# nexus-xyz/nexus-zkvm

Hardware: NVIDIA B200
Metric: RISC-V cycles proved/sec @ 2^20 rows (higher is better)
Workload: dtype u32 (M31)

## Files before the change

### nexus_zkvm_b200/csrc/jit.cu

```cuda
#include "pcs.h"
#include "jit.h"
#include <dlfcn.h>
#include <unistd.h>
#include <cstring>
#include <cstdio>
#include <nvrtc.h>
#include <sstream>
#include <cstdlib>

namespace nb {

static u32 jit_bound() {
  static u32 v = 0;
  if (!v) { v = JIT_BLOCK; if (const char* e = getenv("NB200_JIT_BOUND")) { int x = atoi(e); if (x == 256 || x == 512 || x == 1024) v = (u32)x; } }
  return v;
}


namespace {
struct Nvrtc {
  void* h = nullptr;
  nvrtcResult (*CreateProgram)(nvrtcProgram*, const char*, const char*, int, const char* const*, const char* const*) = nullptr;
  nvrtcResult (*CompileProgram)(nvrtcProgram, int, const char* const*) = nullptr;
  nvrtcResult (*GetCUBINSize)(nvrtcProgram, size_t*) = nullptr;
  nvrtcResult (*GetCUBIN)(nvrtcProgram, char*) = nullptr;
  nvrtcResult (*GetProgramLogSize)(nvrtcProgram, size_t*) = nullptr;
  nvrtcResult (*GetProgramLog)(nvrtcProgram, char*) = nullptr;
  nvrtcResult (*DestroyProgram)(nvrtcProgram*) = nullptr;
  bool ok = false;
};
Nvrtc& nvrtc() {
  static Nvrtc n;
  static bool tried = false;
  if (tried) return n;
  tried = true;
  const char* names[] = {"libnvrtc.so.12", "libnvrtc.so", "/usr/local/cuda/lib64/libnvrtc.so.12"};
  for (const char* nm : names) { n.h = dlopen(nm, RTLD_NOW | RTLD_LOCAL); if (n.h) break; }
  if (!n.h) return n;
#define NB_SYM(f) n.f = (decltype(n.f))dlsym(n.h, "nvrtc" #f); if (!n.f) return n;
  NB_SYM(CreateProgram) NB_SYM(CompileProgram) NB_SYM(GetCUBINSize) NB_SYM(GetCUBIN) NB_SYM(GetProgramLogSize) NB_SYM(GetProgramLog) NB_SYM(DestroyProgram)
#undef NB_SYM
  n.ok = true;
  return n;
}

const char* kPrelude = R"SRC(
typedef unsigned int u32; typedef unsigned long long u64;
#define P31 0x7fffffffu
struct Q { u32 c0, c1, c2, c3; };
__device__ __forceinline__ u32 mn(u32 a, u32 b) { return a < b ? a : b; }
__device__ __forceinline__ u32 add(u32 a, u32 b) { u32 s = a + b; return mn(s, s - P31); }
__device__ __forceinline__ u32 sub(u32 a, u32 b) { u32 d = a - b; return mn(d, d + P31); }
__device__ __forceinline__ u32 neg(u32 a) { return a ? P31 - a : 0u; }
// one product: a * 2b = hi * 2^32 + lo  =>  a * b = hi * 2^31 + lo / 2 == hi + lo / 2 (mod P), below 2P
__device__ __forceinline__ u32 mul2(u32 a, u32 b2) { u64 p = (u64)a * (u64)b2; u32 s = (u32)(p >> 32) + ((u32)p >> 1); return mn(s, s - P31); }
__device__ __forceinline__ u32 mul(u32 a, u32 b) { return mul2(a, b + b); }
// canonical residue of any 64-bit value: 2^32 == 2 and 2^31 == 1 (mod P)
__device__ __forceinline__ u32 red64(u64 x) {
  u64 y;                                                // y = 2 * hi + lo < 3 * 2^32 (mad.wide keeps NVVM from expanding it into a carry chain)
  asm("mad.wide.u32 %0, %1, 2, %2;" : "=l"(y) : "r"((u32)(x >> 32)), "l"((u64)(u32)x));
  u32 yl = (u32)y, yh = (u32)(y >> 32);
  u32 s = (yl & P31) + __funnelshift_r(yl, yh, 31);     // <= P + 5
  return mn(s, s - P31);
}
__device__ __forceinline__ Q qadd(Q x, Q y) { return Q{add(x.c0, y.c0), add(x.c1, y.c1), add(x.c2, y.c2), add(x.c3, y.c3)}; }
__device__ __forceinline__ Q qsub(Q x, Q y) { return Q{sub(x.c0, y.c0), sub(x.c1, y.c1), sub(x.c2, y.c2), sub(x.c3, y.c3)}; }
__device__ __forceinline__ Q qneg(Q x) { return Q{neg(x.c0), neg(x.c1), neg(x.c2), neg(x.c3)}; }
__device__ __forceinline__ Q qmulb(Q x, u32 b) { u32 b2 = b + b; return Q{mul2(x.c0, b2), mul2(x.c1, b2), mul2(x.c2, b2), mul2(x.c3, b2)}; }
__device__ __forceinline__ Q qaddb(Q x, u32 b) { x.c0 = add(x.c0, b); return x; }
__device__ __forceinline__ Q qsubb(Q x, u32 b) { x.c0 = sub(x.c0, b); return x; }
// acc + x * y in QM31 with every coordinate accumulated in 64 bits and reduced once.  (a + bu)(c + du) = (ac + R bd) + (ad + bc)u,
// R = 2 + i (the formula of m31.cuh qm31_mul), regrouped per coordinate of x so that each output is four products:
//   r0 = x0 y0 - x1 y1 + x2 (2 y2 - y3) - x3 (y2 + 2 y3)      r1 = x0 y1 + x1 y0 + x2 (y2 + 2 y3) + x3 (2 y2 - y3)
//   r2 = x0 y2 - x1 y3 + x2 y0 - x3 y1                        r3 = x0 y3 + x1 y2 + x2 y1 + x3 y0
// ny1 = P - y1, ny3 = P - y3, g = 2 y2 - y3, gp = y2 + 2 y3, h = P - gp: all <= P, so 4 products + acc < 2^64.
__device__ __forceinline__ Q qmac(Q acc, Q x, u32 y0, u32 y1, u32 y2, u32 y3, u32 ny1, u32 ny3, u32 g, u32 gp, u32 h) {
  u64 r0 = (u64)acc.c0 + (u64)x.c0 * y0 + (u64)x.c1 * ny1 + (u64)x.c2 * g + (u64)x.c3 * h;
  u64 r1 = (u64)acc.c1 + (u64)x.c0 * y1 + (u64)x.c1 * y0 + (u64)x.c2 * gp + (u64)x.c3 * g;
  u64 r2 = (u64)acc.c2 + (u64)x.c0 * y2 + (u64)x.c1 * ny3 + (u64)x.c2 * y0 + (u64)x.c3 * ny1;
  u64 r3 = (u64)acc.c3 + (u64)x.c0 * y3 + (u64)x.c1 * y2 + (u64)x.c2 * y1 + (u64)x.c3 * y0;
  return Q{red64(r0), red64(r1), red64(r2), red64(r3)};
}
__device__ __forceinline__ Q qmul(Q x, Q y) {
  u32 gp = add(add(y.c3, y.c3), y.c2), g = sub(add(y.c2, y.c2), y.c3);
  return qmac(Q{0u, 0u, 0u, 0u}, x, y.c0, y.c1, y.c2, y.c3, P31 - y.c1, P31 - y.c3, g, gp, P31 - gp);
}
// x^(P-2): 30 squarings + 8 products
__device__ __forceinline__ u32 sqn(u32 x, int n) { for (int i = 0; i < n; ++i) x = mul(x, x); return x; }
__device__ __forceinline__ u32 minv(u32 x) {
  u32 a2 = mul(sqn(x, 1), x), a4 = mul(sqn(a2, 2), a2), a8 = mul(sqn(a4, 4), a4), a16 = mul(sqn(a8, 8), a8);
  u32 a24 = mul(sqn(a16, 8), a8), a28 = mul(sqn(a24, 4), a4), a29 = mul(sqn(a28, 1), x);
  return mul(sqn(a29, 2), x);
}
// (a + bu)^-1 = (a - bu) / (a^2 - (2 + i) b^2), a, b in CM31 (the formula of m31.cuh qm31_inv); the CM31 inverse is conj / norm
__device__ __noinline__ Q qinv(Q q) {
  u32 b2r = sub(mul(q.c2, q.c2), mul(q.c3, q.c3)), b2i = mul(add(q.c2, q.c2), q.c3);           // b^2
  u32 a2r = sub(mul(q.c0, q.c0), mul(q.c1, q.c1)), a2i = mul(add(q.c0, q.c0), q.c1);           // a^2
  u32 dr = sub(a2r, sub(add(b2r, b2r), b2i)), di = sub(a2i, add(add(b2i, b2i), b2r));          // a^2 - (2 b^2 + i b^2)
  u32 ni = minv(add(mul(dr, dr), mul(di, di)));
  u32 ir = mul(dr, ni), ii = neg(mul(di, ni));                                                 // 1 / denom
  return Q{sub(mul(q.c0, ir), mul(q.c1, ii)), add(mul(q.c0, ii), mul(q.c1, ir)),
           neg(sub(mul(q.c2, ir), mul(q.c3, ii))), neg(add(mul(q.c2, ii), mul(q.c3, ir)))};
}
__device__ __forceinline__ Q ldq(const u32* p) { uint4 v = __ldg(reinterpret_cast<const uint4*>(p)); return Q{v.x, v.y, v.z, v.w}; }
// rr + coeff * x with the coefficient's derived multipliers precomputed by the host (12 words per constraint, see jit_coeff_table)
__device__ __forceinline__ Q qmac_tab(Q acc, Q x, const u32* t) {
  uint4 a = __ldg(reinterpret_cast<const uint4*>(t)), b = __ldg(reinterpret_cast<const uint4*>(t) + 1), c = __ldg(reinterpret_cast<const uint4*>(t) + 2);
  return qmac(acc, x, a.x, a.y, a.z, a.w, b.x, b.y, b.z, b.w, c.x);
}
)SRC";

template <class Ld>
void emit_op(std::ostringstream& o, const AirInstr& in, Ld ld) {
  switch (in.op) {
    case OP_LOADM: o << "b[" << in.dst << "] = " << ld(in.a) << ";"; break;
    case OP_CONSTB: o << "b[" << in.dst << "] = " << in.a << "u;"; break;
    case OP_ADDB: o << "b[" << in.dst << "] = add(b[" << in.a << "], b[" << in.b << "]);"; break;
    case OP_SUBB: o << "b[" << in.dst << "] = sub(b[" << in.a << "], b[" << in.b << "]);"; break;
    case OP_MULB: o << "b[" << in.dst << "] = mul(b[" << in.a << "], b[" << in.b << "]);"; break;
    case OP_NEGB: o << "b[" << in.dst << "] = neg(b[" << in.a << "]);"; break;
    case OP_PARAME: o << "e[" << in.dst << "] = ldq(params + " << 4 * in.a << ");"; break;
    case OP_ADDE: o << "e[" << in.dst << "] = qadd(e[" << in.a << "], e[" << in.b << "]);"; break;
    case OP_SUBE: o << "e[" << in.dst << "] = qsub(e[" << in.a << "], e[" << in.b << "]);"; break;
    case OP_MULE: o << "e[" << in.dst << "] = qmul(e[" << in.a << "], e[" << in.b << "]);"; break;
    case OP_NEGE: o << "e[" << in.dst << "] = qneg(e[" << in.a << "]);"; break;
    case OP_ADDEB: o << "e[" << in.dst << "] = qaddb(e[" << in.a << "], b[" << in.b << "]);"; break;
    case OP_SUBEB: o << "e[" << in.dst << "] = qsubb(e[" << in.a << "], b[" << in.b << "]);"; break;
    case OP_MULEB: o << "e[" << in.dst << "] = qmulb(e[" << in.a << "], b[" << in.b << "]);"; break;
    case OP_BTOE: o << "e[" << in.dst << "] = Q{b[" << in.a << "], 0u, 0u, 0u};"; break;
    case OP_LOADME: o << "e[" << in.dst << "] = Q{" << ld(in.a) << ", " << ld(in.a + 1) << ", " << ld(in.a + 2) << ", " << ld(in.a + 3) << "};"; break;
    default: break;
  }
}

struct ChunkLive { std::vector<std::vector<u32>> in_b, in_e, out_b, out_e; };
static void instr_regs(const AirInstr& in, std::vector<u32>& rb, std::vector<u32>& re, int& wb, int& we) {
  wb = we = -1;
  switch (in.op) {
    case OP_LOADM: case OP_CONSTB: wb = (int)in.dst; break;
    case OP_ADDB: case OP_SUBB: case OP_MULB: rb = {in.a, in.b}; wb = (int)in.dst; break;
    case OP_NEGB: rb = {in.a}; wb = (int)in.dst; break;
    case OP_PARAME: case OP_LOADME: we = (int)in.dst; break;
    case OP_ADDE: case OP_SUBE: case OP_MULE: re = {in.a, in.b}; we = (int)in.dst; break;
    case OP_NEGE: re = {in.a}; we = (int)in.dst; break;
    case OP_ADDEB: case OP_SUBEB: case OP_MULEB: re = {in.a}; rb = {in.b}; we = (int)in.dst; break;
    case OP_BTOE: rb = {in.a}; we = (int)in.dst; break;
    case OP_CONSTRB: rb = {in.a}; break;
    case OP_CONSTRE: re = {in.a}; break;
    case OP_FRAC: re = {in.a, in.b}; break;
    default: break;
  }
}
static ChunkLive chunk_liveness(const std::vector<AirInstr>& prog, size_t CH, u32 nb, u32 ne) {
  const size_t n_chunks = (prog.size() + CH - 1) / CH;
  ChunkLive L; L.in_b.resize(n_chunks); L.in_e.resize(n_chunks); L.out_b.resize(n_chunks); L.out_e.resize(n_chunks);
  std::vector<char> lb(nb + 1, 0), le(ne + 1, 0);
  std::vector<std::vector<char>> after_b(n_chunks), after_e(n_chunks);
  for (size_t ci = n_chunks; ci-- > 0;) {
    after_b[ci] = lb; after_e[ci] = le;
    for (size_t pc = std::min(prog.size(), (ci + 1) * CH); pc-- > ci * CH;) {
      std::vector<u32> rb, re; int wb, we;
      instr_regs(prog[pc], rb, re, wb, we);
      if (wb >= 0) lb[wb] = 0;
      if (we >= 0) le[we] = 0;
      for (u32 r : rb) lb[r] = 1;
      for (u32 r : re) le[r] = 1;
    }
    for (u32 r = 0; r < nb; ++r) if (lb[r]) L.in_b[ci].push_back(r);
    for (u32 r = 0; r < ne; ++r) if (le[r]) L.in_e[ci].push_back(r);
  }
  for (size_t ci = 0; ci < n_chunks; ++ci) {
    std::vector<char> wrb(nb + 1, 0), wre(ne + 1, 0);
    for (size_t pc = ci * CH; pc < std::min(prog.size(), (ci + 1) * CH); ++pc) {
      std::vector<u32> rb, re; int wb, we;
      instr_regs(prog[pc], rb, re, wb, we);
      if (wb >= 0) wrb[wb] = 1;
      if (we >= 0) wre[we] = 1;
    }
    for (u32 r = 0; r < nb; ++r) if (wrb[r] && after_b[ci][r]) L.out_b[ci].push_back(r);
    for (u32 r = 0; r < ne; ++r) if (wre[r] && after_e[ci][r]) L.out_e[ci].push_back(r);
  }
  return L;
}

std::string gen_source(const AirComponent& c) {
  std::ostringstream o;
  o << kPrelude;
  const u32 DL = c.log_size;
  o << "__device__ __forceinline__ u32 offrow(u32 i, int off, u32 EL) { const u32 DL = " << DL << ";\n"
    << "  u32 prev = __brev(i) >> (32 - EL); u32 half = 1u << (EL - 1); long long step = (long long)off * (1ll << (EL - DL - 1)); long long v;\n"
    << "  if (prev < half) { v = ((long long)prev + step) % (long long)half; if (v < 0) v += half; }\n"
    << "  else { v = ((long long)prev - step) % (long long)half; if (v < 0) v += half; v += half; }\n"
    << "  return __brev((u32)v) >> (32 - EL); }\n";
  const u32 nb = c.n_base_regs ? c.n_base_regs : 1, ne = c.n_ext_regs ? c.n_ext_regs : 1;
  o << "struct St { u32 b[" << nb << "]; Q e[" << ne << "]; Q rr; };\n";
  o << "#define NB_NMASKS " << c.masks.size() << "\n__constant__ const u32* ccols[NB_NMASKS > 0 ? NB_NMASKS : 1];\n";
  auto ld = [&](u32 m) {
    std::ostringstream s;
    if (c.masks[m].off == 0) s << "__ldg(ccols[" << m << "] + row)";
    else s << "__ldg(ccols[" << m << "] + offrow(row, " << c.masks[m].off << ", EL))";
    return s.str();
  };
  size_t CH = 250;
  if (const char* e = getenv("NB200_JIT_CHUNK")) { long v = atol(e); if (v >= 16 && v <= 100000) CH = (size_t)v; }
  size_t n_chunks = (c.prog.size() + CH - 1) / CH;
  const ChunkLive live = chunk_liveness(c.prog, CH, nb, ne);
  u32 k = 0;
  for (size_t ci = 0; ci < n_chunks; ++ci) {
    o << "__device__ __noinline__ void chunk" << ci << "(St& s, const u32* const* __restrict__ cols, const u32* __restrict__ params, const u32* __restrict__ coeff, u32 row, u32 EL) {\n";
    o << "  u32 b[" << nb << "]; Q e[" << ne << "]; Q rr = s.rr;\n";
    for (u32 r : live.in_b[ci]) o << "  b[" << r << "] = s.b[" << r << "];";
    for (u32 r : live.in_e[ci]) o << "  e[" << r << "] = s.e[" << r << "];";
    o << "\n";
    for (size_t pc = ci * CH; pc < std::min(c.prog.size(), (ci + 1) * CH); ++pc) {
      const AirInstr& in = c.prog[pc];
      o << "  ";
      switch (in.op) {
        case OP_CONSTRB: o << "rr = qadd(rr, qmulb(ldq(coeff + " << JIT_COEFF_WORDS * k << "), b[" << in.a << "]));"; ++k; break;
        case OP_CONSTRE: o << "rr = qmac_tab(rr, e[" << in.a << "], coeff + " << JIT_COEFF_WORDS * k << ");"; ++k; break;
        default: emit_op(o, in, ld); break;
      }
      o << "\n";
    }
    for (u32 r : live.out_b[ci]) o << "  s.b[" << r << "] = b[" << r << "];";
    for (u32 r : live.out_e[ci]) o << "  s.e[" << r << "] = e[" << r << "];";
    o << "\n  s.rr = rr;\n}\n";
  }
  o << "extern \"C\" __global__ void __launch_bounds__(" << jit_bound() << ", 1) nbjit(const u32* const* __restrict__ cols, const u32* __restrict__ params, const u32* __restrict__ coeff,\n"
    << "    const u32* __restrict__ dinv, u32* __restrict__ a0, u32* __restrict__ a1, u32* __restrict__ a2, u32* __restrict__ a3, u32 EL, u32 row0) {\n"
    << "  const u32 row = row0 + blockIdx.x * blockDim.x + threadIdx.x;   // row0: a rank of a multi-GPU proof evaluates its slice of the domain's rows\n  St s;\n"
    << "  for (int i = 0; i < " << nb << "; ++i) s.b[i] = 0u;\n  for (int i = 0; i < " << ne << "; ++i) s.e[i] = Q{0u, 0u, 0u, 0u};\n  s.rr = Q{0u, 0u, 0u, 0u};\n";
  for (size_t ci = 0; ci < n_chunks; ++ci) o << "  chunk" << ci << "(s, cols, params, coeff, row, EL);\n  __syncthreads();\n";
  o << "  const u32 di = __ldg(dinv + (row >> " << DL << "));\n"
    << "  a0[row] = add(a0[row], mul(s.rr.c0, di)); a1[row] = add(a1[row], mul(s.rr.c1, di));\n"
    << "  a2[row] = add(a2[row], mul(s.rr.c2, di)); a3[row] = add(a3[row], mul(s.rr.c3, di));\n}\n";
  return o.str();
}

std::string gen_logup_source(const AirComponent& c) {
  std::ostringstream o;
  o << kPrelude;
  const u32 nb = c.lg_base_regs ? c.lg_base_regs : 1, ne = c.lg_ext_regs ? c.lg_ext_regs : 1;
  o << "struct St { u32 b[" << nb << "]; Q e[" << ne << "]; Q fn, fd, run; };\n";
  o << "#define NB_NMASKS " << c.masks.size() << "\n__constant__ const u32* ccols[NB_NMASKS > 0 ? NB_NMASKS : 1];\n";
  auto ld = [&](u32 m) {
    std::ostringstream s;
    if (m < c.masks.size() && c.masks[m].off == 0 && c.masks[m].tree != 2) s << "__ldg(ccols[" << m << "] + row)";
    else s << "0u";
    return s.str();
  };
  size_t CH = 150;
  size_t n_chunks = (c.logup_prog.size() + CH - 1) / CH;
  const ChunkLive live = chunk_liveness(c.logup_prog, CH, nb, ne);
  const int G = 4;
  u32 k = 0; bool have = false; u32 cur_batch = 0;
  std::vector<u32> pending;
  auto flush = [&](std::ostringstream& o2) {
    const int n = (int)pending.size();
    if (n == 0) return;
    o2 << "  {\n";
    for (int g = 1; g < n; ++g) o2 << "    Q pp" << g << " = qmul(" << (g == 1 ? std::string("pfd0") : "pp" + std::to_string(g - 1)) << ", pfd" << g << ");\n";
    o2 << "    Q iv = qinv(" << (n == 1 ? std::string("pfd0") : "pp" + std::to_string(n - 1)) << ");\n";
    for (int g = n - 1; g >= 1; --g)
      o2 << "    { Q t = qmul(iv, " << (g == 1 ? std::string("pfd0") : "pp" + std::to_string(g - 1)) << "); iv = qmul(iv, pfd" << g << "); pfd" << g << " = t; }\n";
    o2 << "    pfd0 = iv;\n";
    for (int g = 0; g < n; ++g) {
      o2 << "    run = qadd(run, qmul(pfn" << g << ", pfd" << g << "));\n";
      for (int cc = 0; cc < 4; ++cc) o2 << "    out[(" << (4 * (size_t)pending[g] + cc) << "ull << LS) + row] = run.c" << cc << ";\n";
    }
    o2 << "  }\n";
    pending.clear();
  };
  auto finalize = [&](std::ostringstream& o2) {
    o2 << "  pfn" << pending.size() << " = fn; pfd" << pending.size() << " = fd;\n";
    pending.push_back(cur_batch);
    if ((int)pending.size() == G) flush(o2);
  };
  o << "struct Pend { Q n[" << G << "], d[" << G << "]; };\n";
  for (size_t ci = 0; ci < n_chunks; ++ci) {
    o << "__device__ __noinline__ void chunk" << ci << "(St& s, Pend& pe, const u32* const* __restrict__ cols, const u32* __restrict__ params, u32* __restrict__ out, u32 row, u32 LS) {\n";
    o << "  u32 b[" << nb << "]; Q e[" << ne << "]; Q fn = s.fn, fd = s.fd, run = s.run;\n";
    for (int g = 0; g < G; ++g) o << "  Q pfn" << g << " = pe.n[" << g << "], pfd" << g << " = pe.d[" << g << "];\n";
    for (u32 r : live.in_b[ci]) o << "  b[" << r << "] = s.b[" << r << "];";
    for (u32 r : live.in_e[ci]) o << "  e[" << r << "] = s.e[" << r << "];";
    o << "\n";
    for (size_t pc = ci * CH; pc < std::min(c.logup_prog.size(), (ci + 1) * CH); ++pc) {
      const AirInstr& in = c.logup_prog[pc];
      if (in.op == OP_FRAC) {
        u32 bt = c.batching[k];
        if (have && bt != cur_batch) { finalize(o); have = false; }
        if (!have) o << "  fn = e[" << in.a << "]; fd = e[" << in.b << "];\n";
        else o << "  fn = qadd(qmul(fn, e[" << in.b << "]), qmul(e[" << in.a << "], fd)); fd = qmul(fd, e[" << in.b << "]);\n";
        cur_batch = bt; have = true; ++k;
      } else {
        o << "  "; emit_op(o, in, ld); o << "\n";
      }
    }
    if (ci + 1 == n_chunks) { if (have) finalize(o); flush(o); }
    for (u32 r : live.out_b[ci]) o << "  s.b[" << r << "] = b[" << r << "];";
    for (u32 r : live.out_e[ci]) o << "  s.e[" << r << "] = e[" << r << "];";
    o << "\n  s.fn = fn; s.fd = fd; s.run = run;\n";
    for (int g = 0; g < G; ++g) o << "  pe.n[" << g << "] = pfn" << g << "; pe.d[" << g << "] = pfd" << g << ";\n";
    o << "}\n";
  }
  o << "extern \"C\" __global__ void __launch_bounds__(" << JIT_BLOCK << ", 1) nbjit(const u32* const* __restrict__ cols, const u32* __restrict__ params, u32* __restrict__ out, u32 LS) {\n"
    << "  const u32 row = blockIdx.x * blockDim.x + threadIdx.x;\n  St s;\n"
    << "  for (int i = 0; i < " << nb << "; ++i) s.b[i] = 0u;\n  for (int i = 0; i < " << ne << "; ++i) s.e[i] = Q{0u, 0u, 0u, 0u};\n"
    << "  s.fn = Q{0u, 0u, 0u, 0u}; s.fd = Q{1u, 0u, 0u, 0u}; s.run = Q{0u, 0u, 0u, 0u};\n"
    << "  Pend pe; for (int i = 0; i < " << 4 << "; ++i) { pe.n[i] = Q{0u, 0u, 0u, 0u}; pe.d[i] = Q{1u, 0u, 0u, 0u}; }\n";
  for (size_t ci = 0; ci < n_chunks; ++ci) o << "  chunk" << ci << "(s, pe, cols, params, out, row, LS);\n  __syncthreads();\n";
  o << "}\n";
  return o.str();
}
}

std::string jit_source(const AirComponent& c) { return gen_source(c); }
std::string jit_logup_source(const AirComponent& c) { return gen_logup_source(c); }

static u32 jit_block() {
  static u32 b = 0;
  if (!b) { b = 512; if (const char* e = getenv("NB200_JIT_BLOCK")) { int v = atoi(e); if (v == 256 || v == 512 || v == 1024) b = (u32)v; } }
  return b < jit_bound() ? b : jit_bound();
}

bool jit_enabled() {
  const char* e = getenv("NB200_JIT");
  return !(e && e[0] == '0');
}

void jit_release(JitKernel& jk) {
  if (jk.lib) cudaLibraryUnload((cudaLibrary_t)jk.lib);
  jk = JitKernel();
}

static nb200_status jit_compile_source(nb200_ctx* ctx, const AirComponent& c, const std::string& src, JitKernel* out);
nb200_status jit_compile_constraints(nb200_ctx* ctx, const AirComponent& c, JitKernel* out) { return jit_compile_source(ctx, c, gen_source(c), out); }
nb200_status jit_compile_logup(nb200_ctx* ctx, const AirComponent& c, JitKernel* out) { return jit_compile_source(ctx, c, gen_logup_source(c), out); }
uint64_t jit_source_key(const std::string& src) {
  uint64_t h = 1469598103934665603ull;
  auto mix = [&](const char* p, size_t n) { for (size_t i = 0; i < n; ++i) { h ^= (unsigned char)p[i]; h *= 1099511628211ull; } };
  mix(src.data(), src.size());
  const char* tgt = "|sm_100a|nb200-jit-4";
  mix(tgt, strlen(tgt));
  return h;
}
static std::string jit_cache_dir() {
  if (const char* e = getenv("NB200_JIT_CACHE")) return e;
  Dl_info info;
  if (dladdr((const void*)&jit_source_key, &info) && info.dli_fname) {
    std::string p = info.dli_fname;
    size_t k = p.rfind('/');
    return (k == std::string::npos ? std::string(".") : p.substr(0, k)) + "/jit_cache";
  }
  return "";
}
static std::string jit_cache_path(const std::string& src) {
  std::string d = jit_cache_dir();
  if (d.empty()) return "";
  char name[32]; snprintf(name, sizeof name, "/%016llx.cubin", (unsigned long long)jit_source_key(src));
  return d + name;
}
static bool read_file(const std::string& path, std::vector<char>& out) {
  FILE* f = fopen(path.c_str(), "rb");
  if (!f) return false;
  fseek(f, 0, SEEK_END); long n = ftell(f); fseek(f, 0, SEEK_SET);
  bool ok = n > 0;
  if (ok) { out.resize((size_t)n); ok = fread(out.data(), 1, (size_t)n, f) == (size_t)n; }
  fclose(f);
  return ok;
}
static void write_file_atomic(const std::string& path, const std::vector<char>& data) {
  std::string tmp = path + ".tmp" + std::to_string((long)getpid());
  FILE* f = fopen(tmp.c_str(), "wb");
  if (!f) return;
  bool ok = fwrite(data.data(), 1, data.size(), f) == data.size();
  ok = (fclose(f) == 0) && ok;
  if (!ok || rename(tmp.c_str(), path.c_str()) != 0) remove(tmp.c_str());
}
static nb200_status jit_load_cubin(nb200_ctx* ctx, const AirComponent& c, const std::vector<char>& cubin, JitKernel* out) {
  cudaLibrary_t lib;
  cudaError_t e = cudaLibraryLoadData(&lib, cubin.data(), nullptr, nullptr, 0, nullptr, nullptr, 0);
  if (e != cudaSuccess) return set_err(ctx, NB200_ERR_CUDA, std::string("jit: cudaLibraryLoadData: ") + cudaGetErrorString(e));
  cudaKernel_t k;
  e = cudaLibraryGetKernel(&k, lib, "nbjit");
  if (e != cudaSuccess) { cudaLibraryUnload(lib); return set_err(ctx, NB200_ERR_CUDA, std::string("jit: cudaLibraryGetKernel: ") + cudaGetErrorString(e)); }
  out->lib = (void*)lib; out->kernel = (void*)k; out->log_size = c.log_size; out->eval_log = c.eval_log();
  return NB200_OK;
}

static nb200_status jit_compile_source(nb200_ctx* ctx, const AirComponent& c, const std::string& src, JitKernel* out) {
  out->lib = nullptr; out->kernel = nullptr; out->tried = true;
  const std::string cache = jit_cache_path(src);
  if (!cache.empty()) {
    std::vector<char> cubin;
    if (read_file(cache, cubin) && jit_load_cubin(ctx, c, cubin, out) == NB200_OK) return NB200_OK;
    cudaGetLastError();
  }
  Nvrtc& n = nvrtc();
  if (!n.ok) return set_err(ctx, NB200_ERR_STATE, "jit: libnvrtc not available");
  nvrtcProgram prog;
  if (n.CreateProgram(&prog, src.c_str(), "nb200_air.cu", 0, nullptr, nullptr) != NVRTC_SUCCESS) return set_err(ctx, NB200_ERR_STATE, "jit: nvrtcCreateProgram failed");
  const char* opts[] = {"--gpu-architecture=sm_100a", "--std=c++17", "-lineinfo"};
  nvrtcResult r = n.CompileProgram(prog, 3, opts);
  if (r != NVRTC_SUCCESS) {
    size_t ls = 0; n.GetProgramLogSize(prog, &ls);
    std::string log(ls, '\0'); if (ls) n.GetProgramLog(prog, &log[0]);
    n.DestroyProgram(&prog);
    return set_err(ctx, NB200_ERR_STATE, "jit: compile failed: " + log.substr(0, 2000));
  }
  size_t cs = 0; n.GetCUBINSize(prog, &cs);
  std::vector<char> cubin(cs);
  n.GetCUBIN(prog, cubin.data());
  n.DestroyProgram(&prog);
  if (!cache.empty()) write_file_atomic(cache, cubin);
  return jit_load_cubin(ctx, c, cubin, out);
}

void jit_coeff_table(const std::vector<qm31>& coeffs, std::vector<u32>& out) {
  out.assign(coeffs.size() * JIT_COEFF_WORDS, 0u);
  for (size_t k = 0; k < coeffs.size(); ++k) {
    const u32* y = coeffs[k].c;
    u32* t = &out[k * JIT_COEFF_WORDS];
    u32 gp = m31_add(m31_add(y[3], y[3]), y[2]), g = m31_sub(m31_add(y[2], y[2]), y[3]);
    t[0] = y[0]; t[1] = y[1]; t[2] = y[2]; t[3] = y[3];
    t[4] = P31 - y[1]; t[5] = P31 - y[3]; t[6] = g; t[7] = gp; t[8] = P31 - gp;
  }
}

static nb200_status jit_set_cols(nb200_ctx* ctx, const JitKernel& jk, const u32* const* d_cols) {
  void* dptr = nullptr; size_t bytes = 0;
  cudaError_t e = cudaLibraryGetGlobal(&dptr, &bytes, (cudaLibrary_t)jk.lib, "ccols");
  if (e != cudaSuccess) return set_err(ctx, NB200_ERR_CUDA, std::string("jit: cudaLibraryGetGlobal(ccols): ") + cudaGetErrorString(e));
  e = cudaMemcpyAsync(dptr, d_cols, bytes, cudaMemcpyDeviceToDevice, ctx->stream);
  if (e != cudaSuccess) return set_err(ctx, NB200_ERR_CUDA, std::string("jit: ccols copy: ") + cudaGetErrorString(e));
  return NB200_OK;
}

nb200_status jit_launch_logup(nb200_ctx* ctx, const JitKernel& jk, const u32* const* d_cols, const u32* d_params, u32* d_out, u32 log_size) {
  size_t rows = (size_t)1 << log_size;
  if (rows < JIT_BLOCK) return set_err(ctx, NB200_ERR_STATE, "jit: domain too small");
  NB_TRY(jit_set_cols(ctx, jk, d_cols));
  void* args[] = {(void*)&d_cols, (void*)&d_params, (void*)&d_out, (void*)&log_size};
  cudaError_t e = cudaLaunchKernel((const void*)jk.kernel, dim3((u32)(rows / jit_block())), dim3(jit_block()), args, 0, ctx->stream);
  ctx->launches += 1;
  if (e != cudaSuccess) return set_err(ctx, NB200_ERR_CUDA, std::string("jit launch: ") + cudaGetErrorString(e));
  return NB200_OK;
}

nb200_status jit_launch_constraints(nb200_ctx* ctx, const JitKernel& jk, const u32* const* d_cols, const u32* d_params, const u32* d_coeff, const u32* d_dinv, u32* const acc[4],
                                    u32 rows_log, u32 dom_log, u32 row0, size_t n_rows) {
  size_t rows = n_rows ? n_rows : (size_t)1 << rows_log;
  if (rows < JIT_BLOCK || rows % JIT_BLOCK != 0) return set_err(ctx, NB200_ERR_STATE, "jit: row range too small");
  NB_TRY(jit_set_cols(ctx, jk, d_cols));
  u32 el = dom_log;
  u32* a0 = acc[0]; u32* a1 = acc[1]; u32* a2 = acc[2]; u32* a3 = acc[3];
  void* args[] = {(void*)&d_cols, (void*)&d_params, (void*)&d_coeff, (void*)&d_dinv, (void*)&a0, (void*)&a1, (void*)&a2, (void*)&a3, (void*)&el, (void*)&row0};
  cudaError_t e = cudaLaunchKernel((const void*)jk.kernel, dim3((u32)(rows / jit_block())), dim3(jit_block()), args, 0, ctx->stream);
  ctx->launches += 1;
  if (e != cudaSuccess) return set_err(ctx, NB200_ERR_CUDA, std::string("jit launch: ") + cudaGetErrorString(e));
  return NB200_OK;
}

}
```

Measured before the change: 15.03 million.

## Fold constraint coefficients into JIT expression trees and specialize logup numerators

Adds an SSA pass over the constraint program that finds constraints of the form (mul - base) whose denominator subtree is linear in parameters and base lifts. For these it pushes the random coefficient into the leaves: per-block shared-memory precomputed coeff*param values, coefficient-scaled base lifts, and a plain add at the sink instead of a full extension multiply. In the logup kernel, numerators that are base lifts or constants become base-field scalings, adds or subtracts instead of full extension multiplies. offrow is also rewritten with masking in place of 64-bit modulo. The goal is fewer extension-field multiplies per row. The cost is an extra shared-memory init and sync per block, plus more complex code generation that could be wrong for unusual program shapes.

```diff
diff --git a/nexus_zkvm_b200/csrc/jit.cu b/nexus_zkvm_b200/csrc/jit.cu
--- a/nexus_zkvm_b200/csrc/jit.cu
+++ b/nexus_zkvm_b200/csrc/jit.cu
@@ -7,6 +7,8 @@
 #include <nvrtc.h>
 #include <sstream>
 #include <cstdlib>
+#include <map>
+#include <algorithm>
 
 namespace nb {
 
@@ -183,15 +185,96 @@
   return L;
 }
 
+struct Ssa { std::vector<int> a, b, uses; };
+static Ssa ssa_rename(const std::vector<AirInstr>& prog, u32 nb, u32 ne) {
+  Ssa s; s.a.assign(prog.size(), -1); s.b.assign(prog.size(), -1); s.uses.assign(prog.size(), 0);
+  std::vector<int> cb(nb + 1, -1), ce(ne + 1, -1);
+  for (size_t pc = 0; pc < prog.size(); ++pc) {
+    const AirInstr& in = prog[pc];
+    switch (in.op) {
+      case OP_ADDB: case OP_SUBB: case OP_MULB: s.a[pc] = cb[in.a]; s.b[pc] = cb[in.b]; break;
+      case OP_NEGB: case OP_BTOE: case OP_CONSTRB: s.a[pc] = cb[in.a]; break;
+      case OP_ADDE: case OP_SUBE: case OP_MULE: case OP_FRAC: s.a[pc] = ce[in.a]; s.b[pc] = ce[in.b]; break;
+      case OP_NEGE: case OP_CONSTRE: s.a[pc] = ce[in.a]; break;
+      case OP_ADDEB: case OP_SUBEB: case OP_MULEB: s.a[pc] = ce[in.a]; s.b[pc] = cb[in.b]; break;
+      default: break;
+    }
+    if (s.a[pc] >= 0) ++s.uses[s.a[pc]];
+    if (s.b[pc] >= 0) ++s.uses[s.b[pc]];
+    std::vector<u32> rb, re; int wb, we;
+    instr_regs(in, rb, re, wb, we);
+    if (wb >= 0) cb[wb] = (int)pc;
+    if (we >= 0) ce[we] = (int)pc;
+  }
+  return s;
+}
+
+enum FoldKind : uint8_t { FOLD_NONE, FOLD_PARAM, FOLD_BTOE, FOLD_EB, FOLD_SUBCONST, FOLD_SUBBASE, FOLD_SINK };
+struct Fold { std::vector<uint8_t> kind; std::vector<u32> k, slot; std::vector<std::pair<u32, u32>> scaled; };
+static bool fold_scalable(const std::vector<AirInstr>& prog, const Ssa& s, int v) {
+  if (v < 0 || s.uses[v] != 1) return false;
+  switch (prog[v].op) {
+    case OP_PARAME: case OP_BTOE: return true;
+    case OP_MULEB: case OP_NEGE: case OP_ADDEB: case OP_SUBEB: return fold_scalable(prog, s, s.a[v]);
+    case OP_ADDE: case OP_SUBE: return fold_scalable(prog, s, s.a[v]) && fold_scalable(prog, s, s.b[v]);
+    case OP_MULE: return fold_scalable(prog, s, s.a[v]) || fold_scalable(prog, s, s.b[v]);
+    default: return false;
+  }
+}
+static void fold_apply(const std::vector<AirInstr>& prog, const Ssa& s, int v, u32 k, Fold& f, std::map<std::pair<u32, u32>, u32>& slots) {
+  switch (prog[v].op) {
+    case OP_PARAME: {
+      auto key = std::make_pair(k, prog[v].a);
+      auto it = slots.find(key);
+      if (it == slots.end()) { it = slots.emplace(key, (u32)f.scaled.size()).first; f.scaled.push_back(key); }
+      f.kind[v] = FOLD_PARAM; f.slot[v] = it->second; break;
+    }
+    case OP_BTOE: f.kind[v] = FOLD_BTOE; break;
+    case OP_ADDEB: case OP_SUBEB: f.kind[v] = FOLD_EB; fold_apply(prog, s, s.a[v], k, f, slots); break;
+    case OP_MULEB: case OP_NEGE: fold_apply(prog, s, s.a[v], k, f, slots); break;
+    case OP_ADDE: case OP_SUBE: fold_apply(prog, s, s.a[v], k, f, slots); fold_apply(prog, s, s.b[v], k, f, slots); break;
+    case OP_MULE: fold_apply(prog, s, fold_scalable(prog, s, s.a[v]) ? s.a[v] : s.b[v], k, f, slots); break;
+    default: break;
+  }
+  f.k[v] = k;
+}
+static Fold fold_coefficients(const AirComponent& c, u32 nb, u32 ne) {
+  const std::vector<AirInstr>& prog = c.prog;
+  const Ssa s = ssa_rename(prog, nb, ne);
+  Fold f; f.kind.assign(prog.size(), FOLD_NONE); f.k.assign(prog.size(), 0); f.slot.assign(prog.size(), 0);
+  std::map<std::pair<u32, u32>, u32> slots;
+  u32 k = 0;
+  for (size_t pc = 0; pc < prog.size(); ++pc) {
+    if (prog[pc].op == OP_CONSTRB) { ++k; continue; }
+    if (prog[pc].op != OP_CONSTRE) continue;
+    const int x = s.a[pc];
+    if (x >= 0 && s.uses[x] == 1 && prog[x].op == OP_SUBE) {
+      const int t = s.a[x], n = s.b[x];
+      if (t >= 0 && s.uses[t] == 1 && prog[t].op == OP_MULE && n >= 0 && prog[n].op == OP_BTOE) {
+        const int den = fold_scalable(prog, s, s.b[t]) ? s.b[t] : fold_scalable(prog, s, s.a[t]) ? s.a[t] : -1;
+        if (den >= 0) {
+          fold_apply(prog, s, den, k, f, slots);
+          const int nb_def = s.a[n];
+          if (nb_def >= 0 && prog[nb_def].op == OP_CONSTB) { f.kind[x] = FOLD_SUBCONST; f.slot[x] = prog[nb_def].a; }
+          else f.kind[x] = FOLD_SUBBASE;
+          f.k[x] = k;
+          f.kind[pc] = FOLD_SINK;
+        }
+      }
+    }
+    ++k;
+  }
+  return f;
+}
+
 std::string gen_source(const AirComponent& c) {
   std::ostringstream o;
   o << kPrelude;
   const u32 DL = c.log_size;
   o << "__device__ __forceinline__ u32 offrow(u32 i, int off, u32 EL) { const u32 DL = " << DL << ";\n"
-    << "  u32 prev = __brev(i) >> (32 - EL); u32 half = 1u << (EL - 1); long long step = (long long)off * (1ll << (EL - DL - 1)); long long v;\n"
-    << "  if (prev < half) { v = ((long long)prev + step) % (long long)half; if (v < 0) v += half; }\n"
-    << "  else { v = ((long long)prev - step) % (long long)half; if (v < 0) v += half; v += half; }\n"
-    << "  return __brev((u32)v) >> (32 - EL); }\n";
+    << "  u32 prev = __brev(i) >> (32 - EL); u32 half = 1u << (EL - 1); u32 step = (u32)off << (EL - DL - 1);\n"
+    << "  u32 v = prev < half ? ((prev + step) & (half - 1)) : (((prev - step) & (half - 1)) | half);\n"
+    << "  return __brev(v) >> (32 - EL); }\n";
   const u32 nb = c.n_base_regs ? c.n_base_regs : 1, ne = c.n_ext_regs ? c.n_ext_regs : 1;
   o << "struct St { u32 b[" << nb << "]; Q e[" << ne << "]; Q rr; };\n";
   o << "#define NB_NMASKS " << c.masks.size() << "\n__constant__ const u32* ccols[NB_NMASKS > 0 ? NB_NMASKS : 1];\n";
@@ -205,6 +288,15 @@
   if (const char* e = getenv("NB200_JIT_CHUNK")) { long v = atol(e); if (v >= 16 && v <= 100000) CH = (size_t)v; }
   size_t n_chunks = (c.prog.size() + CH - 1) / CH;
   const ChunkLive live = chunk_liveness(c.prog, CH, nb, ne);
+  const Fold fold = fold_coefficients(c, nb, ne);
+  const size_t NS = fold.scaled.size();
+  o << "#ifndef __CUDACC__\n#define __shared__ static\n#endif\n#define NB_NSCALED " << NS << "\n__shared__ Q scp[NB_NSCALED > 0 ? NB_NSCALED : 1];\n";
+  if (NS) {
+    o << "__constant__ const u32 scp_src[" << 2 * NS << "] = {";
+    for (size_t i = 0; i < NS; ++i) o << (i ? "," : "") << fold.scaled[i].first << "," << fold.scaled[i].second;
+    o << "};\n";
+  }
+  auto cq = [&](u32 kk) { return "ldq(coeff + " + std::to_string(JIT_COEFF_WORDS * kk) + ")"; };
   u32 k = 0;
   for (size_t ci = 0; ci < n_chunks; ++ci) {
     o << "__device__ __noinline__ void chunk" << ci << "(St& s, const u32* const* __restrict__ cols, const u32* __restrict__ params, const u32* __restrict__ coeff, u32 row, u32 EL) {\n";
@@ -217,8 +309,27 @@
       o << "  ";
       switch (in.op) {
         case OP_CONSTRB: o << "rr = qadd(rr, qmulb(ldq(coeff + " << JIT_COEFF_WORDS * k << "), b[" << in.a << "]));"; ++k; break;
-        case OP_CONSTRE: o << "rr = qmac_tab(rr, e[" << in.a << "], coeff + " << JIT_COEFF_WORDS * k << ");"; ++k; break;
-        default: emit_op(o, in, ld); break;
+        case OP_CONSTRE:
+          if (fold.kind[pc] == FOLD_SINK) o << "rr = qadd(rr, e[" << in.a << "]);";
+          else o << "rr = qmac_tab(rr, e[" << in.a << "], coeff + " << JIT_COEFF_WORDS * k << ");";
+          ++k; break;
+        default:
+          switch (fold.kind[pc]) {
+            case FOLD_PARAM: o << "e[" << in.dst << "] = scp[" << fold.slot[pc] << "];"; break;
+            case FOLD_BTOE: o << "e[" << in.dst << "] = qmulb(" << cq(fold.k[pc]) << ", b[" << in.a << "]);"; break;
+            case FOLD_SUBCONST:
+              if (fold.slot[pc] == 1) o << "e[" << in.dst << "] = qsub(e[" << in.a << "], " << cq(fold.k[pc]) << ");";
+              else o << "e[" << in.dst << "] = qsub(e[" << in.a << "], qmulb(" << cq(fold.k[pc]) << ", " << fold.slot[pc] << "u));";
+              break;
+            case FOLD_SUBBASE:
+              o << "e[" << in.dst << "] = qsub(e[" << in.a << "], qmulb(" << cq(fold.k[pc]) << ", e[" << in.b << "].c0));";
+              break;
+            case FOLD_EB:
+              o << "e[" << in.dst << "] = " << (in.op == OP_ADDEB ? "qadd" : "qsub") << "(e[" << in.a << "], qmulb(" << cq(fold.k[pc]) << ", b[" << in.b << "]));";
+              break;
+            default: emit_op(o, in, ld); break;
+          }
+          break;
       }
       o << "\n";
     }
@@ -230,6 +341,9 @@
     << "    const u32* __restrict__ dinv, u32* __restrict__ a0, u32* __restrict__ a1, u32* __restrict__ a2, u32* __restrict__ a3, u32 EL, u32 row0) {\n"
     << "  const u32 row = row0 + blockIdx.x * blockDim.x + threadIdx.x;   // row0: a rank of a multi-GPU proof evaluates its slice of the domain's rows\n  St s;\n"
     << "  for (int i = 0; i < " << nb << "; ++i) s.b[i] = 0u;\n  for (int i = 0; i < " << ne << "; ++i) s.e[i] = Q{0u, 0u, 0u, 0u};\n  s.rr = Q{0u, 0u, 0u, 0u};\n";
+  if (NS)
+    o << "  for (u32 i = threadIdx.x; i < NB_NSCALED; i += blockDim.x) scp[i] = qmul(ldq(coeff + " << JIT_COEFF_WORDS << " * scp_src[2 * i]), ldq(params + 4 * scp_src[2 * i + 1]));\n"
+      << "  __syncthreads();\n";
   for (size_t ci = 0; ci < n_chunks; ++ci) o << "  chunk" << ci << "(s, cols, params, coeff, row, EL);\n  __syncthreads();\n";
   o << "  const u32 di = __ldg(dinv + (row >> " << DL << "));\n"
     << "  a0[row] = add(a0[row], mul(s.rr.c0, di)); a1[row] = add(a1[row], mul(s.rr.c1, di));\n"
@@ -253,8 +367,29 @@
   size_t n_chunks = (c.logup_prog.size() + CH - 1) / CH;
   const ChunkLive live = chunk_liveness(c.logup_prog, CH, nb, ne);
   const int G = 4;
+  std::vector<int> num_kind(c.batching.size(), 0);
+  std::vector<u32> num_const(c.batching.size(), 0);
+  {
+    const Ssa ss = ssa_rename(c.logup_prog, nb, ne);
+    std::vector<int> batch_len(c.batching.empty() ? 0 : *std::max_element(c.batching.begin(), c.batching.end()) + 1, 0);
+    for (u32 bt : c.batching) ++batch_len[bt];
+    u32 kf = 0;
+    for (size_t pc = 0; pc < c.logup_prog.size(); ++pc) {
+      if (c.logup_prog[pc].op != OP_FRAC) continue;
+      const int n = ss.a[pc];
+      if (batch_len[c.batching[kf]] == 1 && n >= 0 && c.logup_prog[n].op == OP_BTOE) {
+        const int bd = ss.a[n];
+        if (bd >= 0 && c.logup_prog[bd].op == OP_CONSTB) {
+          const u32 v = c.logup_prog[bd].a;
+          num_kind[kf] = v == 1 ? 2 : v == P31 - 1 ? 3 : 4; num_const[kf] = v;
+        } else num_kind[kf] = 1;
+      }
+      ++kf;
+    }
+  }
   u32 k = 0; bool have = false; u32 cur_batch = 0;
   std::vector<u32> pending;
+  std::vector<u32> pending_frac;
   auto flush = [&](std::ostringstream& o2) {
     const int n = (int)pending.size();
     if (n == 0) return;
@@ -265,15 +400,23 @@
       o2 << "    { Q t = qmul(iv, " << (g == 1 ? std::string("pfd0") : "pp" + std::to_string(g - 1)) << "); iv = qmul(iv, pfd" << g << "); pfd" << g << " = t; }\n";
     o2 << "    pfd0 = iv;\n";
     for (int g = 0; g < n; ++g) {
-      o2 << "    run = qadd(run, qmul(pfn" << g << ", pfd" << g << "));\n";
+      const u32 f = pending_frac[g];
+      switch (num_kind[f]) {
+        case 1: o2 << "    run = qadd(run, qmulb(pfd" << g << ", pfn" << g << ".c0));\n"; break;
+        case 2: o2 << "    run = qadd(run, pfd" << g << ");\n"; break;
+        case 3: o2 << "    run = qsub(run, pfd" << g << ");\n"; break;
+        case 4: o2 << "    run = qadd(run, qmulb(pfd" << g << ", " << num_const[f] << "u));\n"; break;
+        default: o2 << "    run = qadd(run, qmul(pfn" << g << ", pfd" << g << "));\n"; break;
+      }
       for (int cc = 0; cc < 4; ++cc) o2 << "    out[(" << (4 * (size_t)pending[g] + cc) << "ull << LS) + row] = run.c" << cc << ";\n";
     }
     o2 << "  }\n";
-    pending.clear();
+    pending.clear(); pending_frac.clear();
   };
   auto finalize = [&](std::ostringstream& o2) {
-    o2 << "  pfn" << pending.size() << " = fn; pfd" << pending.size() << " = fd;\n";
-    pending.push_back(cur_batch);
+    if (num_kind[k - 1] >= 2) o2 << "  pfd" << pending.size() << " = fd;\n";
+    else o2 << "  pfn" << pending.size() << " = fn; pfd" << pending.size() << " = fd;\n";
+    pending.push_back(cur_batch); pending_frac.push_back(k - 1);
     if ((int)pending.size() == G) flush(o2);
   };
   o << "struct Pend { Q n[" << G << "], d[" << G << "]; };\n";
@@ -340,7 +483,7 @@
   uint64_t h = 1469598103934665603ull;
   auto mix = [&](const char* p, size_t n) { for (size_t i = 0; i < n; ++i) { h ^= (unsigned char)p[i]; h *= 1099511628211ull; } };
   mix(src.data(), src.size());
-  const char* tgt = "|sm_100a|nb200-jit-4";
+  const char* tgt = "|sm_100a|nb200-jit-5";
   mix(tgt, strlen(tgt));
   return h;
 }
```

Result: faster. 15.46 million, median of 6 (+2.9%).
